# cslab-ntua/sparsex

Measured on AMD Instinct MI355X. Metric: SpMV GFLOP/s (2*nnz/t, alpha=0.5, x/y resident in HBM), higher is better.
Workload: dtype f64

## Files before the change

### include/sparsex_hip.h

```cpp
#ifndef SPARSEX_HIP_H
#define SPARSEX_HIP_H

#include <sparsex/sparsex.h>
#include <stdint.h>

#ifdef __cplusplus
extern "C" {
#endif

spx_error_t spx_hip_matvec_mult(spx_value_t alpha, const spx_matrix_t *A,
                                const spx_value_t *x_dev, spx_value_t *y_dev,
                                void *stream);
spx_error_t spx_hip_matvec_kernel(spx_value_t alpha, const spx_matrix_t *A,
                                  const spx_value_t *x_dev, spx_value_t beta,
                                  spx_value_t *y_dev, void *stream);

spx_error_t spx_hip_matvec_trans_mult(spx_value_t alpha, const spx_matrix_t *A,
                                      const spx_value_t *x_dev, spx_value_t *y_dev,
                                      void *stream);
spx_error_t spx_hip_matvec_trans_kernel(spx_value_t alpha, const spx_matrix_t *A,
                                        const spx_value_t *x_dev, spx_value_t beta,
                                        spx_value_t *y_dev, void *stream);
int spx_hip_matvec_trans_mode(const spx_matrix_t *A);

// ... 125 lines not shown
int spx_hip_mat_dist_parts(const spx_matrix_t *A);
spx_error_t spx_hip_mat_dist_round(const spx_matrix_t *A, int round, const size_t **send_off, const size_t **send_cnt,
                                   const size_t **recv_off, const size_t **recv_cnt);

typedef struct {
    int64_t nnz;
    int64_t nnz_stored;
    int64_t n_unit_elems;
    int64_t n_delta_elems;
    int64_t n_units;
    int64_t n_rowblocks;
    int64_t n_shared_rows;
    int64_t value_bytes;
    int64_t index_bytes;
    int32_t nr_partitions;
    int32_t first_partition, last_partition;
    int32_t row_lo, row_hi;
    int32_t symmetric;
    int32_t on_device;
    int32_t device;
    int32_t waves;
    int32_t sym_tiles;
    double  tune_seconds;
    double  emit_seconds;
    int32_t wave_tiles;
    int32_t sym_segments;
    int32_t quad;
    int32_t col_slices;
    int32_t unit_windows;
    int32_t unit_window_lds;
    int64_t unit_window_elems;
    int64_t unit_window_staged;
    int32_t sym_pipeline;
    int32_t reserved0;
    int64_t sym_pipeline_elems;
} spx_hip_info_t;

spx_error_t spx_hip_mat_info(const spx_matrix_t *A, spx_hip_info_t *info);

typedef struct {
    const uint32_t *tab;
    const uint32_t *xdescs;
    const void *passes;
    size_t n_rowblocks, n_descs, n_passes;
    size_t rowblocks_with_windows, rowblocks_with_units;
    uint64_t staged_doubles;
    uint64_t unit_elems, unit_elems_lds;
    uint32_t lds_doubles;
} spx_hip_xw_plan_t;
spx_error_t spx_hip_mat_unit_windows(spx_matrix_t *A, uint32_t budget, uint32_t gap, spx_hip_xw_plan_t *plan);

typedef struct {
    const void *passes;
    const uint32_t *n_sx;
    size_t n_rowblocks, n_passes;
    size_t rowblocks_with_sx;
    uint64_t sym_elems, sx_elems;
    uint64_t sym_passes, sx_passes;
} spx_hip_sx_plan_t;
spx_error_t spx_hip_mat_sym_pipeline(spx_matrix_t *A, spx_hip_sx_plan_t *plan);

spx_error_t spx_hip_mat_values_plan(spx_matrix_t *A, const spx_index_t *rowptr, const spx_index_t *colind, int indexing);
spx_error_t spx_hip_mat_values_plan_drop(spx_matrix_t *A);
spx_error_t spx_hip_mat_set_values(spx_matrix_t *A, const spx_value_t *values_dev, void *stream);
spx_error_t spx_hip_mat_set_values_host(spx_matrix_t *A, const spx_value_t *values);
typedef struct {
    const uint32_t *src_values;
// ... 65 lines not shown
```

### sparsex_amd/api.py

```python
import ctypes as C
import os

import numpy as np

SPX_SUCCESS = 0
SPX_FAILURE = -1
SPX_MAT_REORDER = 42
SPX_VEC_AS_IS = 43
SPX_VEC_TUNE = 44
SPX_INDEX_ZERO_BASED = 45
SPX_INDEX_ONE_BASED = 46

_HERE = os.path.dirname(os.path.abspath(__file__))


def lib_path():
    return os.environ.get("SPX_LIB_PATH") or os.path.join(_HERE, "lib", "libsparsex.so")


class SpxError(RuntimeError):
    pass


class VectorStruct(C.Structure):
    _fields_ = [("elements", C.POINTER(C.c_double)), ("size", C.c_size_t),
                ("alloc_type", C.c_int), ("vec_mode", C.c_int)]


class HipInfo(C.Structure):
    _fields_ = [("nnz", C.c_int64), ("nnz_stored", C.c_int64),
                ("n_unit_elems", C.c_int64), ("n_delta_elems", C.c_int64),
                ("n_units", C.c_int64), ("n_rowblocks", C.c_int64),
                ("n_shared_rows", C.c_int64), ("value_bytes", C.c_int64),
                ("index_bytes", C.c_int64), ("nr_partitions", C.c_int32),
                ("first_partition", C.c_int32), ("last_partition", C.c_int32),
                ("row_lo", C.c_int32), ("row_hi", C.c_int32),
                ("symmetric", C.c_int32), ("on_device", C.c_int32),
                ("device", C.c_int32), ("waves", C.c_int32), ("sym_tiles", C.c_int32),
                ("tune_seconds", C.c_double),
                ("emit_seconds", C.c_double), ("wave_tiles", C.c_int32), ("sym_segments", C.c_int32),
                ("quad", C.c_int32), ("col_slices", C.c_int32),
                ("unit_windows", C.c_int32), ("unit_window_lds", C.c_int32),
                ("unit_window_elems", C.c_int64), ("unit_window_staged", C.c_int64),
                ("sym_pipeline", C.c_int32), ("reserved0", C.c_int32), ("sym_pipeline_elems", C.c_int64)]


class SxPlan(C.Structure):
    _fields_ = [("passes", C.c_void_p), ("n_sx", C.POINTER(C.c_uint32)), ("n_rowblocks", C.c_size_t),
                ("n_passes", C.c_size_t), ("rowblocks_with_sx", C.c_size_t), ("sym_elems", C.c_uint64),
                ("sx_elems", C.c_uint64), ("sym_passes", C.c_uint64), ("sx_passes", C.c_uint64)]


class ValuesPlan(C.Structure):
    _fields_ = [("src_values", C.POINTER(C.c_uint32)), ("src_mirror", C.POINTER(C.c_uint32)),
                ("src_diag", C.POINTER(C.c_uint32)), ("n_values", C.c_size_t), ("n_mirror", C.c_size_t),
                ("n_diag", C.c_size_t), ("n_sources", C.c_uint64), ("n_dest", C.c_uint64),
                ("plan_bytes", C.c_uint64)]


class DiagPlan(C.Structure):
    _fields_ = [("pos", C.POINTER(C.c_uint32)), ("n_rows", C.c_size_t), ("row_lo", C.c_size_t),
                ("n_present", C.c_uint64), ("plan_bytes", C.c_uint64)]


class XwPlan(C.Structure):
    _fields_ = [("tab", C.POINTER(C.c_uint32)), ("xdescs", C.POINTER(C.c_uint32)), ("passes", C.c_void_p),
                ("n_rowblocks", C.c_size_t), ("n_descs", C.c_size_t), ("n_passes", C.c_size_t),
                ("rowblocks_with_windows", C.c_size_t), ("rowblocks_with_units", C.c_size_t),
                ("staged_doubles", C.c_uint64), ("unit_elems", C.c_uint64), ("unit_elems_lds", C.c_uint64),
                ("lds_doubles", C.c_uint32)]


class CsxExport(C.Structure):
    _fields_ = [("values", C.POINTER(C.c_double)), ("ctl", C.POINTER(C.c_uint8)),
                ("ctl_size", C.c_int64), ("nnz", C.c_int), ("ncols", C.c_int),
                ("nrows", C.c_int), ("row_start", C.c_int),
                ("row_jumps", C.c_int32), ("full_colind", C.c_int32),
# ... 999 lines not shown
```

### sparsex_amd/csrc/api.cpp

```cpp
#include <sparsex/sparsex.h>
#include <sparsex_hip.h>

#include "config.hpp"
#include "csx_emit.hpp"
#include "device.hpp"
#include "dist.hpp"
#include "encoder.hpp"
#include "gpu_emit.hpp"
#include "input.hpp"
#include "reorder.hpp"
#include "stream_index.hpp"
#include "threads.hpp"

#include <chrono>
#include <cmath>
#include <cstdarg>
#include <cstdint>
#include <cstring>
#include <functional>
#include <memory>
#include <mutex>
#include <atomic>
#include <sstream>
#include <thread>
// ... 333 lines not shown
{
    for (const SpxRowBlock &rb : s.rbs)
        for (uint32_t k = 0; k < rb.n_pass; ++k) {
            const uint8_t kind = s.passes[(size_t) rb.pass_off + k].kind;
            if (kind == SPX_PASS_SYMTILE || kind == SPX_PASS_SYMSEG) return true;
        }
    return false;
}

static void keep_index(spx_matrix_t *A, GpuStream &&gs)
{
    ValVec().swap(gs.values);
    std::vector<val_t>().swap(gs.dvalues);
    std::vector<val_t>().swap(gs.mirror_val);
    std::vector<uint32_t>().swap(gs.fix_idx);
    std::vector<uint32_t>().swap(gs.fix_ptr);
    std::vector<uint32_t>().swap(gs.spill_col);
    A->index.reset(new GpuStream(std::move(gs)));
}

constexpr size_t JOINED_ROWS = 1024, JOINED_ELEMS = 24576;
constexpr uint32_t JOINED_XW_BUDGET = 8192;

static size_t auto_target_elems(const spx_matrix_t *A, double scale)
{
    size_t local = 0;
    for (const Partition &p : A->parts) local += p.nnz * (A->symmetric ? 2 : 1);
    size_t t = std::min<size_t>(std::max<size_t>(local / 1280 + 1, 1024),
                                local > ((size_t) 64 << 20) ? SPX_MAX_RB_ELEMS : 4096);
    t = std::max<size_t>((size_t)(scale * (double) t), 512);
    return std::min<size_t>(t, SPX_MAX_RB_ELEMS);
}

static void emit_and_upload(spx_matrix_t *A)
{
    const size_t nown = A->parts.size();
    const size_t first = A->first_part;
    const bool sym = A->symmetric != 0;
    GpuEmitParams gp = A->emit_params;
    if (A->auto_rb) gp.target_elems = auto_target_elems(A, A->rb_scale);
    if (A->rb_joined) {
        gp.target_elems = JOINED_ELEMS;
        gp.max_rows = std::max<size_t>(gp.max_rows, JOINED_ROWS);
    }
    GpuStream gs;
    const unsigned hw = host_threads();
    struct Deferred {
        std::function<void()> f;
        ~Deferred() { if (f) f(); }
    } deferred;
    std::function<void()> &release_after_upload = deferred.f;
    const double t_emit0 = now_sec();
    auto emit_pieces = [&](std::vector<Partition> &pieces, const std::vector<std::vector<SymTile>> *tl,
                           const std::vector<SymSegVec> *sl = nullptr) {
        const size_t n = pieces.size();
        std::vector<GpuStream> locs(n);
        const unsigned inner = (unsigned) std::max<size_t>(1, hw / std::max<size_t>(1, std::min<size_t>(n, hw)));
        const double t_pieces = now_sec();
        parallel_for(n, hw, [&](size_t i) {
            GpuEmitParams g = gp;
            if (tl) g.tiles = &(*tl)[i];
            if (sl) g.symsegs = &(*sl)[i];
            emit_gpu(pieces[i], g, locs[i], inner);
        });
        const double t_room = now_sec();
        std::vector<uint64_t> v_at(n, UINT64_MAX);
        {
            size_t nv = gs.values.size(), nd = gs.descs.size(), np = gs.passes.size(), nc = gs.cidx.size(),
                   ns = gs.segrows.size(), nr = gs.rbs.size();
            for (size_t i = 0; i < n; ++i) {
                const GpuStream &l = locs[i];
                if (!(l.rbs.empty() && l.shared.empty())) {
                    nv += nv % 2;
                    v_at[i] = nv;
                    nv += l.values.size();
                }
// ... 138 lines not shown
                q.nr_rows = p.nr_rows; q.nr_cols = p.nr_cols; q.type = p.type; q.row_start = p.row_start;
                q.pool = p.pool;
                for (size_t e = 0; e < p.elems_size; ++e)
                    if (p.elems[e].col >= c_lo && p.elems[e].col < c_hi) {
                        q.elems.push_back(p.elems[e]);
                        q.nnz += p.elems[e].size;
                    }
                q.elems_size = q.elems.size();
            });
            gp.skip_empty = k > 0 || A->col_concurrent;
            const size_t rb0 = gs.rbs.size();
            emit_pieces(sub, nullptr);
            if (k > 0 && gs.rbs.size() > rb0) gs.rbs[rb0].flags |= SPX_RB_PHASE_START;
            if (A->col_concurrent && gs.rbs.size() == rb0) throw FatalError("column phases: an empty slice");
        }
        if (A->col_concurrent)
            for (SpxRowBlock &rb : gs.rbs) rb.flags |= SPX_RB_ACCUM;
        gp = keep;
        if (!gs.shared.empty()) throw FatalError("column phases: the matrix holds rows that are split over row-blocks");
    }
    const double t_emit1 = now_sec();
    A->conflict_rows.clear();
    if (sym && !gs.sym_fused) stream_touched_rows(gs, A->own_lo, A->conflict_rows);
    A->halo_cols.clear();
    if (A->own_lo > 0 || A->own_hi < A->nrows) stream_read_cols(gs, A->own_lo, A->own_hi, (size_t) A->ncols, A->halo_cols);
    A->first_block_row = A->own_lo;
    for (const SpxRowBlock &rb : gs.rbs) A->first_block_row = std::min<idx_t>(A->first_block_row, (idx_t) rb.row0);
    finalize_stream(gs, (size_t) A->nrows);
    if (sym) mark_private_rowblocks(gs, (size_t) A->nrows, A->own_lo, A->own_hi);
    std::vector<std::pair<uint32_t, uint32_t>>().swap(gs.direct_cols);
    gs.waves = (uint32_t) A->waves;
    gs.band_order = Config::instance().get_bool("spx.gpu.band_order");
    gs.arena = Config::instance().get_bool("spx.gpu.arena");
    gs.xw_budget = (A->unit_windows != 0 && !A->deterministic && !sym) ? (A->rb_joined ? std::max(A->xw_budget, JOINED_XW_BUDGET) : A->xw_budget) : 0u;
    gs.xw_gap = A->xw_gap;
    gs.xw_on = A->xw_on;
    gs.sx_plan = sym && A->sym_pipeline != 0 && !A->deterministic && A->wave_tiles != 1;
    gs.sx_on = A->sx_on;
    gs.sym_matmat = A->sym_matmat;
    gs.sym_atomic = A->sym_atomic && !A->deterministic;
    gs.deterministic = A->deterministic;
    gs.wave_tiles = A->deterministic || A->wave_tiles == 1;
    A->nnz_stored = gs.nnz_stored;
    A->n_unit_elems = gs.n_unit_elems;
    A->n_delta_elems = gs.n_delta_elems;
    A->n_units = gs.n_units;
    A->value_bytes = gs.values.size() * sizeof(val_t);
    A->index_bytes = gs.index_bytes();
    A->n_rowblocks = gs.rbs.size();
    A->n_shared = gs.shared.size();
    A->has_tiles = stream_has_tiles(gs);
    A->has_symtiles = stream_has_pass(gs, SPX_PASS_SYMTILE);
    if (A->dev) {
        device_free(A->dev);
        A->dev = nullptr;
    }
    const double t_emit2 = now_sec();
    if (!A->host_only) {
        A->dev = device_upload(gs, (size_t) A->nrows, (size_t) A->ncols, sym, A->own_lo, A->own_hi,
                               A->device_ordinal);
        device_set_trans_windows(A->dev, A->trans_windows);
        log_msg(LOG_INFO, "descriptor stream: emitted in %.2f s, finalized in %.2f s, uploaded in %.2f s (%zu row-blocks)\n",
                t_emit1 - t_emit0, t_emit2 - t_emit1, now_sec() - t_emit2, gs.rbs.size());
        if (A->dist && sym) {
            device_set_init_rows(A->dev, (size_t) dist_first_init_row(*A));
        }
        keep_index(A, std::move(gs));
// ... 17 lines not shown
    auto best_time = [&]() {
        A->release_wait();
        double best = device_time_spmv(A->dev, W, N);
        for (int rep = 0; rep < 3; ++rep) best = std::min(best, device_time_spmv(A->dev, 0, N));
        return best;
    };
    auto time_xw = [&](bool &xw) {
        if (!tune_xw || !device_has_xw(A->dev) || A->wave_tiles == 1) {
            xw = device_get_xw(A->dev);
            return best_time();
        }
        device_set_xw(A->dev, false);
        const double t0 = best_time();
        device_set_xw(A->dev, true);
        const double t1 = best_time();
        xw = t1 < 0.985 * t0;
        device_set_xw(A->dev, xw);
        return std::min(t0, xw ? t1 : t0);
    };
    if (!tune_waves) {
        if (tune_wave_tiles && !device_has_tiles(A->dev) && !(A->unit_windows == 1 && device_has_xw(A->dev))) {
            auto t_of = [&](bool on) {
                device_set_wave_tiles(A->dev, on);
                return best_time();
            };
            const double t0 = t_of(false), t1 = t_of(true);
            A->wave_tiles = t1 < 0.985 * t0 ? 1 : 0;
            device_set_wave_tiles(A->dev, A->wave_tiles == 1);
        }
        if (tune_xw && device_has_xw(A->dev) && A->wave_tiles != 1) {
            bool xw = false;
            (void) time_xw(xw);
            A->xw_on = xw;
        }
        if (!tune_spill || !device_has_spill(A->dev)) return;
        auto t_of = [&](bool atomic) {
            device_set_sym_atomic(A->dev, atomic);
            return best_time();
        };
        const double tl = t_of(false), ta = t_of(true);
        A->sym_atomic = ta < 0.985 * tl;
        device_set_sym_atomic(A->dev, A->sym_atomic);
        return;
    }
    auto time_with = [&](int waves, bool &xw) {
        device_set_waves(A->dev, waves);
        return time_xw(xw);
    };
    bool xw4 = false, xw8 = false;
    const double t4 = time_with(4, xw4), t8 = time_with(8, xw8);
    int best_waves = t8 < 0.985 * t4 ? 8 : 4;
    bool best_xw = best_waves == 8 ? xw8 : xw4;
    double best_t = std::min(t4, t8), best_scale = 1.0;
    device_set_xw(A->dev, best_xw);
    A->xw_on = best_xw;
    if (tune_wave_tiles && !device_has_tiles(A->dev) && !(A->unit_windows == 1 && device_has_xw(A->dev))) {
        device_set_wave_tiles(A->dev, true);
        device_set_waves(A->dev, best_waves);
        const double tw = best_time();
        if (tw < 0.985 * best_t) {
            best_t = tw;
            A->wave_tiles = 1;
            best_xw = false;
            A->xw_on = false;
        } else {
            device_set_wave_tiles(A->dev, false);
// ... 3 lines not shown
    }
    if (tune_spill && device_has_spill(A->dev)) {
        device_set_sym_atomic(A->dev, !A->sym_atomic);
        device_set_waves(A->dev, best_waves);
        const double ta = best_time();
        if (ta < 0.985 * best_t) {
            best_t = ta;
            A->sym_atomic = !A->sym_atomic;
        } else {
            device_set_sym_atomic(A->dev, A->sym_atomic);
        }
    }
    if (A->auto_rb && A->n_rowblocks <= 4096) {
        for (double scale : {0.7, 0.52}) {
            A->rb_scale = scale;
            A->waves = 2;
            emit_and_upload(A);
            bool xw2 = false;
            const double t2 = time_with(2, xw2);
            if (t2 < 0.985 * best_t) {
                best_t = t2;
                best_waves = 2;
                best_scale = scale;
                best_xw = xw2;
            }
        }
        A->xw_on = best_xw;
        if (A->rb_scale != best_scale) {
            A->rb_scale = best_scale;
            A->waves = best_waves;
            emit_and_upload(A);
        }
    }
    if (A->auto_rb && A->n_rowblocks > 4096 &&
        auto_target_elems(A, 2.0) != auto_target_elems(A, best_scale)) {
        A->rb_scale = 2.0;
        A->waves = best_waves;
        emit_and_upload(A);
        bool xwb = false;
        const double tb = time_with(best_waves, xwb);
        if (tb < 0.985 * best_t) {
            best_t = tb;
            best_scale = 2.0;
            best_xw = xwb;
            A->xw_on = best_xw;
        } else {
            A->rb_scale = best_scale;
            A->xw_on = best_xw;
            emit_and_upload(A);
        }
    }
    A->rb_scale = best_scale;
    A->waves = best_waves;
    A->xw_on = best_xw;
    if (A->auto_rb && best_xw && A->wave_tiles != 1 && A->emit_params.max_rows <= SPX_MAX_RB_ROWS &&
        A->value_bytes > ((size_t) 1 << 30)) {
        A->rb_joined = true;
        A->waves = 8;
        emit_and_upload(A);
        bool xwj = false;
        const double tj = time_with(8, xwj);
        if (xwj && tj < 0.995 * best_t) {
            best_t = tj;
            best_waves = 8;
            log_msg(LOG_INFO, "launch autotune: row-blocks joined side by side (%zu of them)\n", A->n_rowblocks);
        } else {
            A->rb_joined = false;
            A->waves = best_waves;
            A->xw_on = best_xw;
            emit_and_upload(A);
        }
    }
    A->waves = best_waves;
    A->xw_on = best_xw;
    device_set_waves(A->dev, best_waves);
    device_set_xw(A->dev, best_xw);
    log_msg(LOG_INFO, "launch autotune: %d wavefronts per workgroup, row-block scale %.2f%s, unit windows %s (%.2f us per SpMV)\n",
            best_waves, best_scale, A->rb_joined ? ", joined" : "", best_xw ? "on" : "off", 1e6 * best_t);
}

static int read_trans_windows()
{
    const std::string tw = Config::instance().get_str("spx.gpu.trans_windows");
    if (tw != "auto" && tw != "true" && tw != "false") {
        log_msg(LOG_ERR, "spx.gpu.trans_windows: true, false or auto\n");
        throw FatalError("bad spx.gpu.trans_windows");
    }
    return tw == "auto" ? -1 : (tw == "true" ? 1 : 0);
}

static int read_values_f32()
{
    const std::string v = Config::instance().get_str("spx.gpu.values_f32");
    if (v != "true" && v != "false" && v != "all") {
        log_msg(LOG_ERR, "spx.gpu.values_f32: false, true or all\n");
        throw FatalError("bad spx.gpu.values_f32");
    }
    return v == "all" ? 2 : (v == "true" ? 1 : 0);
}
static bool wants_values_f32(int mode, bool symmetric) { return mode == 2 || (mode == 1 && !symmetric); }

static spx_matrix_t *do_tune(spx_input_t *in)
{
    Config &cfg = Config::instance();
    const double t0 = now_sec();
    const size_t P = cfg.nr_partitions();
    long world = std::max<long>(1, cfg.get_long("spx.rt.gpu_world"));
    long rank = cfg.get_long("spx.rt.gpu_rank");
    if (rank < 0 || rank >= world || P % (size_t) world != 0) {
        log_msg(LOG_ERR, "spx.rt.gpu_rank/gpu_world (%ld/%ld) do not divide "
                "spx.rt.nr_threads=%zu partitions\n", rank, world, P);
// ... 183 lines not shown
        log_msg(LOG_ERR, "spx.gpu.unit_windows: true, false or auto\n");
        throw FatalError("bad spx.gpu.unit_windows");
    }
    {
        const long xb = cfg.get_long("spx.gpu.unit_window_doubles"), xg = cfg.get_long("spx.gpu.unit_window_gap");
        if (xb < 0 || xb > 16384 || xg < 0 || xg > 255) {
            log_msg(LOG_ERR, "spx.gpu.unit_window_doubles: 0 .. 16384, spx.gpu.unit_window_gap: 0 .. 255\n");
            throw FatalError("bad spx.gpu.unit_window_doubles / spx.gpu.unit_window_gap");
        }
        A->xw_budget = (uint32_t) xb;
        A->xw_gap = (uint32_t) xg;
    }
    A->unit_windows = xw_mode == "auto" ? -1 : (xw_mode == "true" ? 1 : 0);
    A->xw_on = xw_mode == "true";
    A->trans_windows = read_trans_windows();
    A->values_f32 = read_values_f32();
    const std::string sx_mode = cfg.get_str("spx.gpu.sym_pipeline");
    if (sx_mode != "auto" && sx_mode != "true" && sx_mode != "false") {
        log_msg(LOG_ERR, "spx.gpu.sym_pipeline: true, false or auto\n");
        throw FatalError("bad spx.gpu.sym_pipeline");
    }
    A->sym_pipeline = sx_mode == "auto" ? -1 : (sx_mode == "true" ? 1 : 0);
    A->sx_on = sx_mode == "true";
    const std::string ph_mode = cfg.get_str("spx.gpu.col_phases");
    const bool ph_conc = ph_mode.size() == 2 && ph_mode[0] == 'c';
    long ph_fixed = ph_mode == "auto" ? 0 : strtol(ph_mode.c_str() + (ph_conc ? 1 : 0), nullptr, 10);
    if (ph_mode != "auto" && (ph_fixed < 1 || ph_fixed > 8 || (ph_conc && ph_fixed != 2 && ph_fixed != 4 && ph_fixed != 8))) {
        log_msg(LOG_ERR, "spx.gpu.col_phases: 1 .. 8 (launched in turn), c2 | c4 | c8 (one launch, a group of XCDs each) or auto\n");
        throw FatalError("bad spx.gpu.col_phases");
    }
    A->col_phases = (!sym && ph_fixed > 1) ? (size_t) ph_fixed : 1;
    A->col_concurrent = A->col_phases > 1 && ph_conc && !A->deterministic;
    if (A->col_phases > 1 && ph_conc && !A->col_concurrent) A->col_phases = 1;
    try {
        emit_and_upload(A.get());
    } catch (const FatalError &) {
        if (A->col_phases <= 1) throw;
        A->col_phases = 1;
        emit_and_upload(A.get());
    }
    const bool tune_spill = spill_mode == "auto" && !A->deterministic && !A->has_symsegs && !A->sym_matmat;
    const bool tune_wt = wt_mode == "auto" && !A->deterministic && !A->has_symsegs;
    const bool tune_xw = xw_mode == "auto" && !A->deterministic && !sym;
    const double t_auto = now_sec();
    if (A->dev && A->nnz_stored >= 100000 && (autotune || tune_spill || tune_wt || tune_xw))
        autotune_launch(A.get(), autotune, tune_spill, tune_wt, tune_xw);
    if (A->dev && sym && A->sym_pipeline == -1 && device_has_sx(A->dev)) {
        A->release_wait();
        const double t_est = device_time_spmv(A->dev, 2, 3);
        const int N = (int) std::min(100.0, std::max(8.0, 0.02 / std::max(t_est, 1e-7)));
        auto best_of = [&](bool on) {
            device_set_sx(A->dev, on);
            double best = device_time_spmv(A->dev, std::max(2, N / 10), N);
            for (int rep = 0; rep < 3; ++rep) best = std::min(best, device_time_spmv(A->dev, 0, N));
            return best;
        };
        const double t0 = best_of(false), t1 = best_of(true);
        A->sx_on = t1 < 0.985 * t0;
        device_set_sx(A->dev, A->sx_on);
        log_msg(LOG_INFO, "read-once pipeline: %s (%.2f us per SpMV with, %.2f without)\n", A->sx_on ? "on" : "off", 1e6 * t1, 1e6 * t0);
    }
    const double t_auto_end = now_sec();
    if (A->dev && !sym && ph_mode == "auto" && A->n_shared == 0 && A->nnz_stored >= 100000 &&
        2 * A->n_delta_elems >= A->nnz_stored && (size_t) A->ncols * sizeof(val_t) >= ((size_t) 6 << 20)) {
        auto best_of = [&]() {
            double best = device_time_spmv(A->dev, 10, 100);
// ... 1420 lines not shown
} SPX_C_BOUNDARY(return SPX_FAILURE;)

spx_error_t spx_hip_mat_info(const spx_matrix_t *A, spx_hip_info_t *info)
try {
    if (!A || !info) { SETERROR_1(SPX_ERR_ARG_INVALID, "invalid argument"); return SPX_FAILURE; }
    memset(info, 0, sizeof(*info));
    info->nnz = A->nnz;
    info->nnz_stored = (int64_t) A->nnz_stored;
    info->n_unit_elems = (int64_t) A->n_unit_elems;
    info->n_delta_elems = (int64_t) A->n_delta_elems;
    info->n_units = (int64_t) A->n_units;
    info->n_rowblocks = (int64_t) A->n_rowblocks;
    info->n_shared_rows = (int64_t) A->n_shared;
    info->value_bytes = (int64_t) A->value_bytes;
    info->index_bytes = (int64_t) A->index_bytes;
    info->nr_partitions = (int32_t) A->nr_partitions;
    info->first_partition = (int32_t) A->first_part;
    info->last_partition = (int32_t) A->last_part;
    info->row_lo = A->own_lo;
    info->row_hi = A->own_hi;
    info->symmetric = A->symmetric;
    info->on_device = A->dev ? 1 : 0;
    if (A->dev) {
        DeviceMatrixInfo di;
        device_info(A->dev, di);
        info->device = di.device;
    }
    info->waves = A->dev ? device_get_waves(A->dev) : A->waves;
    info->sym_tiles = A->has_tiles ? ((A->dev ? device_get_sym_atomic(A->dev) : A->sym_atomic) ? 2 : 1) : 0;
    info->wave_tiles = A->dev ? (device_get_wave_tiles(A->dev) ? 1 : 0) : (A->wave_tiles == 1 || A->deterministic ? 1 : 0);
    info->sym_segments = A->has_symsegs ? (A->has_symtiles ? 1 : 2) : 0;
    info->col_slices = A->col_phases > 1 ? (A->col_concurrent ? (int32_t) A->col_phases : -(int32_t) A->col_phases) : 1;
    info->quad = 0;
    if (A->dev && device_has_xw(A->dev)) {
        uint64_t el = 0, ue = 0, st = 0;
        uint32_t lds = 0;
        device_xw_info(A->dev, el, ue, st, lds);
        info->unit_windows = device_get_xw(A->dev) ? 1 : 0;
        info->unit_window_lds = (int32_t) lds;
        info->unit_window_elems = (int64_t) el;
        info->unit_window_staged = (int64_t) st;
    }
    if (A->dev && device_has_sx(A->dev)) {
        uint64_t esx = 0, esym = 0;
        size_t nrb = 0;
        device_sx_info(A->dev, esx, esym, nrb);
        info->sym_pipeline = device_get_sx(A->dev) ? 1 : 0;
        info->sym_pipeline_elems = (int64_t) esx;
    }
    info->tune_seconds = A->tune_seconds;
    info->emit_seconds = A->emit_seconds;
    return SPX_SUCCESS;
} SPX_C_BOUNDARY(return SPX_FAILURE;)

static bool owned_part(const spx_matrix_t *A, int part)
{
    return part >= (int) A->first_part && part < (int) A->last_part &&
           (size_t)(part - (int) A->first_part) < A->parts.size();
}

spx_error_t spx_hip_mat_export_csx(const spx_matrix_t *A_, int part, spx_csx_export_t *out)
try {
    spx_matrix_t *A = const_cast<spx_matrix_t *>(A_);
    if (!A || !out) { SETERROR_1(SPX_ERR_ARG_INVALID, "invalid argument"); return SPX_FAILURE; }
    if (!owned_part(A, part)) {
        SETERROR_1(SPX_ERR_ARG_INVALID, "partition not held by this process "
// ... 323 lines not shown
```

### sparsex_amd/csrc/config.cpp

```cpp
#include "config.hpp"

#include <cstdlib>
#include <regex>
#include <sstream>

namespace spx {

Config &Config::instance()
{
    static Config c;
    return c;
}

Config::Config() { reset_defaults(); }

void Config::reset_defaults()
{
    props_.clear();
    props_["spx.rt.nr_threads"] = "1";
    props_["spx.rt.cpu_affinity"] = "0";
    props_["spx.preproc.heuristic"] = "ratio";
    props_["spx.preproc.xform"] = "all";
    props_["spx.preproc.sampling"] = "portion";
    props_["spx.preproc.sampling.nr_samples"] = "48";
    props_["spx.preproc.sampling.portion"] = "0.01";
    props_["spx.preproc.sampling.window_size"] = "0";
    props_["spx.matrix.symmetric"] = "false";
    props_["spx.matrix.split_blocks"] = "true";
    props_["spx.matrix.full_colind"] = "false";
    props_["spx.matrix.min_unit_size"] = "4";
    props_["spx.matrix.max_unit_size"] = "255";
    props_["spx.matrix.min_coverage"] = "0.1";
    props_["spx.matrix.onedim_blocks"] = "false";
    props_["spx.rt.host_only"] = "false";
    props_["spx.rt.gpu_rank"] = "0";
    props_["spx.rt.gpu_world"] = "1";
    props_["spx.rt.device"] = "-1";
    props_["spx.vec.register"] = "auto";
    props_["spx.vec.device"] = "false";
    props_["spx.rt.host_parts"] = "0";
    props_["spx.rt.dist_chunks"] = "4";
    props_["spx.rt.dist_reorder"] = "none";
    props_["spx.rt.row_offset"] = "0";
    props_["spx.rt.global_rows"] = "0";
    props_["spx.rt.keep_encoded"] = "true";
    props_["spx.gpu.rowblock_elems"] = "0";
    props_["spx.gpu.rowblock_rows"] = "512";
    props_["spx.gpu.stack_segments"] = "true";
    props_["spx.gpu.waves"] = "0";
    props_["spx.gpu.inline_desc"] = "true";
    props_["spx.gpu.arena"] = "false";
    props_["spx.gpu.band_order"] = "false";
    props_["spx.gpu.col_phases"] = "auto";
    props_["spx.gpu.keep_units"] = "true";
    props_["spx.gpu.recut_linear"] = "true";
    props_["spx.gpu.sym_once"] = "true";
    props_["spx.gpu.deterministic"] = "false";
    props_["spx.gpu.wave_tiles"] = "auto";
    props_["spx.gpu.x_window"] = "true";
    props_["spx.gpu.sym_segments"] = "auto";
    props_["spx.gpu.sym_segment_min"] = "2";
    props_["spx.gpu.sym_segment_max"] = "8";
    props_["spx.gpu.sym_wide_rows"] = "1024";
    props_["spx.gpu.sym_spill"] = "auto";
    props_["spx.gpu.sym_matmat"] = "false";
    props_["spx.gpu.sym_remine"] = "true";
    props_["spx.gpu.sym_pure_passes"] = "true";
    props_["spx.gpu.sym_pipeline"] = "auto";
    props_["spx.gpu.unit_windows"] = "auto";
    props_["spx.gpu.unit_window_doubles"] = "3072";
    props_["spx.gpu.unit_window_gap"] = "16";
    props_["spx.gpu.values_f32"] = "false";
    props_["spx.gpu.trans_windows"] = "auto";
}

bool Config::set(const std::string &key, const std::string &value)
{
    auto it = props_.find(key);
    if (it == props_.end()) {
        log_msg(LOG_WARN, "mnemonic \"%s\" not found\n", key.c_str());
// ... 138 lines not shown
```

### sparsex_amd/csrc/gpu_emit.cpp

```cpp
#include "gpu_emit.hpp"
#include "threads.hpp"

#include <algorithm>
#include <iterator>
#include <cassert>
#include <cstring>
#include <chrono>

namespace spx {

namespace {

struct Piece {
    uint32_t elem;
    uint16_t a, b;
};

struct Single { idx_t row, col; val_t val; };
typedef std::vector<Single, BigAlloc<Single>> SingleVec;
struct RowSeg { idx_t row, col; uint8_t width; val_t v[SPX_MAX_SEG_WIDTH]; };

template <class V, class KeyOf, class Within>
void sort_by_key_then(V &v, KeyOf key_of, Within within)
{
// ... 1237 lines not shown
    for (size_t i = 0; i < s.rbs.size(); ++i) {
        SpxRowBlock &rb = s.rbs[i];
        std::copy(s.passes.begin() + rb.pass_off, s.passes.begin() + rb.pass_off + rb.n_pass,
                  strided.begin() + i * (size_t) stride);
        rb.pass_off = (uint32_t)(i * (size_t) stride);
    }
    s.passes.swap(strided);
    s.pass_stride = stride;
}

void mark_private_rowblocks(GpuStream &s, size_t nrows, idx_t own_lo, idx_t own_hi)
{
    std::vector<char> touched(nrows + 8, 0);
    for (uint32_t g : s.slot_group_col)
        for (uint32_t c = g; c < g + 8; ++c) touched[c] = 1;
    for (const auto &d : s.direct_cols)
        for (uint32_t c = d.first; c < d.first + d.second && c < nrows; ++c) touched[c] = 1;
    for (uint32_t r : s.mirror_rows) touched[r] = 1;
    std::vector<uint32_t> upto(nrows + 1, 0);
    for (size_t r = 0; r < nrows; ++r) upto[r + 1] = upto[r] + (touched[r] ? 1u : 0u);
    for (SpxRowBlock &rb : s.rbs) {
        rb.flags &= (uint8_t) ~SPX_RB_PRIVATE;
        const size_t lo = rb.row0, hi = (size_t) rb.row0 + rb.n_rows;
        if ((rb.flags & SPX_RB_SHARED) || (idx_t) lo < own_lo || (idx_t) hi > own_hi || hi > nrows) continue;
        if (upto[hi] == upto[lo]) rb.flags |= SPX_RB_PRIVATE;
    }
}

void emit_gpu(const Partition &p, const GpuEmitParams &prm, GpuStream &out, unsigned nthreads)
{
    assert(p.type == ENC_H);
    const idx_t nrows = (idx_t) p.nr_rows;
    if (nrows == 0) return;
    const size_t max_rows = std::min<size_t>(prm.max_rows, SPX_MAX_RB_ROWS);
    const size_t target = std::min<size_t>(std::max<size_t>(prm.target_elems, 64),
                                           SPX_MAX_RB_ELEMS);

    std::vector<uint32_t> cnt((size_t) nrows, 0);
    for (size_t i = 0; i < p.elems_size; ++i) {
        const Elem &e = p.elems[i];
        if (!e.is_unit()) { ++cnt[(size_t) e.row - 1]; continue; }
        for (size_t k = 0; k < e.size; ++k) {
            idx_t r, c;
            unit_elem_coords(e, k, r, c);
            assert(r >= 1 && r <= nrows);
            ++cnt[(size_t) r - 1];
        }
    }
    static const std::vector<SymTile> no_tiles;
    const std::vector<SymTile> &tiles = prm.tiles ? *prm.tiles : no_tiles;
    for (const SymTile &t : tiles)
        for (idx_t r = 0; r < 8; ++r) cnt[(size_t)(t.row0 - p.row_start + r)] += 8;
    static const SymSegVec no_segs;
    const SymSegVec &symsegs = prm.symsegs ? *prm.symsegs : no_segs;
    for (const SymSeg &sg : symsegs) cnt[(size_t)(sg.row - p.row_start)] += sg.width;

    std::vector<char> tile_group((size_t) nrows / 8 + 2, 0);
    const idx_t g0 = p.row_start / 8;
    for (const SymTile &t : tiles) tile_group[(size_t)(t.row0 / 8 - g0)] = 1;
    auto in_group = [&](idx_t r) { return tile_group[(size_t)((p.row_start + r) / 8 - g0)] != 0; };
    std::vector<Plan> plans;
    {
        idx_t start = 0;
        size_t acc = 0;
        for (idx_t r = 0; r < nrows; ++r) {
            size_t c = cnt[(size_t) r];
            if (c > SPX_MAX_RB_ELEMS) {
                if (in_group(r)) throw FatalError("symmetric tile on an over-long row");
// ... 170 lines not shown
            }
            a = b;
        }
    };

    std::vector<std::vector<const SymTile *>> rb_tiles(plans.size());
    for (const SymTile &t : tiles) {
        const size_t r = (size_t)(t.row0 - p.row_start);
        const uint32_t pl = plan_of_row[r];
        if (plan_of_row[r + 7] != pl || plans[pl].split)
            throw FatalError("symmetric tile cut by a row-block border");
        rb_tiles[pl].push_back(&t);
    }

    std::vector<std::vector<const SymSeg *>> rb_segs(plans.size());
    for (const SymSeg &sg : symsegs) {
        const uint32_t pl = plan_of_row[(size_t)(sg.row - p.row_start)];
        if (plans[pl].split) throw FatalError("read-once segment on an over-long row");
        rb_segs[pl].push_back(&sg);
    }

    std::vector<std::pair<size_t, size_t>> jobs;
    {
        const size_t wide_seg = std::min<size_t>(prm.wide_rows, SPX_MAX_WIDE_ROWS);
        const size_t wide_any = std::min<size_t>(prm.max_rows, SPX_MAX_WIDE_ROWS);
        auto elems_of = [&](size_t i) {
            size_t e = 0;
            for (idx_t r = plans[i].row_lo; r < plans[i].row_hi; ++r) e += cnt[(size_t) r];
            return e;
        };
        auto joinable = [&](size_t i, bool seg) {
            if (plans[i].split || !rb_tiles[i].empty()) return false;
            return seg ? wide_seg > SPX_MAX_RB_ROWS && !rb_segs[i].empty()
                       : wide_any > SPX_MAX_RB_ROWS && rb_segs[i].empty();
        };
        for (size_t i = 0; i < plans.size();) {
            size_t j = i + 1;
            if (joinable(i, true)) {
                const idx_t row0g = p.row_start + plans[i].row_lo;
                auto seg_groups = [&](size_t q, std::vector<idx_t> &g) {
                    g.clear();
                    for (const SymSeg *sg : rb_segs[q])
                        for (idx_t c = sg->col & ~(idx_t) 7; c < sg->col + sg->width && c < row0g; c += 8) g.push_back(c);
                    std::sort(g.begin(), g.end());
                    g.erase(std::unique(g.begin(), g.end()), g.end());
                };
                std::vector<idx_t> uni, g, merged;
                seg_groups(i, uni);
                while (j < plans.size() && joinable(j, true) &&
                       (size_t)(plans[j].row_hi - plans[i].row_lo) <= wide_seg) {
                    seg_groups(j, g);
                    merged.clear();
                    std::set_union(uni.begin(), uni.end(), g.begin(), g.end(), std::back_inserter(merged));
                    if (merged.size() * 8 > SPX_MAX_WIDE_SLOTS) break;
                    uni.swap(merged);
                    ++j;
                }
            } else if (joinable(i, false)) {
                size_t e = elems_of(i);
                const size_t join_target = std::max<size_t>(target, std::min<size_t>(prm.target_elems, 4 * SPX_MAX_RB_ELEMS));
                while (j < plans.size() && joinable(j, false) &&
                       (size_t)(plans[j].row_hi - plans[i].row_lo) <= wide_any &&
                       e + elems_of(j) <= join_target + elems_of(j) / 2) {
                    e += elems_of(j);
                    ++j;
                }
            }
// ... 65 lines not shown
```

### sparsex_amd/csrc/gpu_emit.hpp

```cpp
#pragma once

#include "gpu_format.h"
#include "partition.hpp"

#include <utility>
#include <vector>

namespace spx {

struct SymTile {
    idx_t row0, col0;
    val_t v[64];
};

struct SymSeg {
    idx_t row, col;
    uint8_t width;
    val_t v[8];
};
typedef std::vector<SymSeg, BigAlloc<SymSeg>> SymSegVec;

struct GpuStream {
    ValVec values;
    std::vector<SpxUnitDesc> descs;
// ... 19 lines not shown
    uint32_t n_spill = 0;
    uint32_t lds_doubles = SPX_MAX_RB_ROWS;
    uint32_t pass_stride = 0;
    uint32_t waves = 4;
    bool band_order = false;
    bool arena = false;
    uint32_t xw_budget = 0, xw_gap = 16;
    bool xw_on = false;
    bool sx_plan = false, sx_on = false;
    bool sym_matmat = false;
    size_t nnz_stored = 0;
    size_t n_unit_elems = 0;
    size_t n_delta_elems = 0;
    size_t n_units = 0;

    size_t n_pass_used() const
    {
        size_t n = 0;
        for (const SpxRowBlock &rb : rbs) n += rb.n_pass;
        return n;
    }
    size_t index_bytes() const
    {
        return descs.size() * sizeof(SpxUnitDesc) + n_pass_used() * sizeof(SpxPass) + cidx.size() +
               (sym_atomic ? slot_group_col.size() : fix_ptr.size() + fix_idx.size()) * 4 +
               (mirror_rows.size() + mirror_ptr.size() + mirror_col.size()) * 4 +
               segrows.size() * 2 + rbs.size() * sizeof(SpxRowBlock);
    }
};

struct GpuEmitParams {
    size_t target_elems = 2048;
    size_t max_rows = SPX_MAX_RB_ROWS;
    size_t sym_min_run = 2;
    size_t sym_max_run = SPX_MAX_SEG_WIDTH;
    size_t wide_rows = SPX_MAX_RB_ROWS;
    bool skip_empty = false;
    bool stack_segments = true;
    bool recut_linear = true;
    bool inline_desc = true;
    bool keep_units = true;
    bool sym_remine = true;
    bool x_window = true;
    int sym_segments = -1;
    bool sym_pure_passes = true;
    bool sym_once = true;
    const std::vector<SymTile> *tiles = nullptr;
    const SymSegVec *symsegs = nullptr;
};

void emit_gpu(const Partition &p, const GpuEmitParams &prm, GpuStream &out, unsigned nthreads = 1);

void append_stream(GpuStream &dst, GpuStream &&src, uint64_t values_placed_at = UINT64_MAX);

void finalize_stream(GpuStream &s, size_t nrows);

void mark_private_rowblocks(GpuStream &s, size_t nrows, idx_t own_lo, idx_t own_hi);

void append_sym_expanded(const Partition &lower, Partition &out, bool remine_upper = true);

struct SymRange { idx_t lo, hi; };
struct MirrorPoint { idx_t row, col; val_t val; };
void build_sym_ranges(const std::vector<Partition> &lowers, const std::vector<SymRange> &ranges,
                      bool want_tiles, std::vector<Partition> &outs,
                      std::vector<std::vector<SymTile>> &tiles, unsigned nthreads,
                      std::vector<MirrorPoint> *sparse_mirror = nullptr,
// ... 24 lines not shown
```

### sparsex_amd/csrc/handles.hpp

```cpp
#pragma once

#include <sparsex/sparsex.h>
#include <sparsex_hip.h>

#include "csx_emit.hpp"
#include "device.hpp"
#include "gpu_emit.hpp"
#include "input.hpp"
#include "xwindows.hpp"
#include "sxplan.hpp"
#include "values_plan.hpp"
#include "diag_plan.hpp"

#include <algorithm>
#include <functional>
#include <memory>
#include <mutex>
#include <string>
#include <vector>
#include <thread>

namespace spx { struct DistPlan; }

using namespace spx;
// ... 39 lines not shown
    }
    ~matrix() { release_wait(); }
    std::vector<std::vector<val_t>> diag;
    std::vector<std::unique_ptr<CsxStream>> exported;
    std::vector<std::vector<spx_index_t>> exported_rows_info;
    bool full_colind = false;
    DeviceMatrix *dev = nullptr;
    std::unique_ptr<GpuStream> host_stream;
    std::unique_ptr<GpuStream> index;
    idx_t own_lo = 0, own_hi = 0;
    std::vector<idx_t> conflict_rows;
    std::vector<idx_t> halo_cols;
    idx_t first_block_row = 0;
    spx::DistPlan *dist = nullptr;
    GpuEmitParams emit_params;
    bool auto_rb = false;
    double rb_scale = 1.0;
    int waves = 4;
    size_t col_phases = 1;
    bool col_concurrent = false;
    bool host_only = false;
    bool has_tiles = false;
    bool sym_atomic = false;
    bool deterministic = false;
    bool has_symtiles = false;
    bool has_symsegs = false;
    int spill_mode = -1;
    bool sym_matmat = false;
    int wave_tiles = -1;
    int unit_windows = -1;
    bool xw_on = false;
    int values_f32 = 0;
    int trans_windows = -1;
    bool rb_joined = false;
    int sym_pipeline = -1;
    bool sx_on = false;
    uint32_t xw_budget = 3072, xw_gap = 16;
    std::unique_ptr<spx::XwPlan> xw_inspect;
    std::unique_ptr<spx::SxPlan> sx_inspect;
    std::unique_ptr<spx::ValuesPlan> values_plan;
    size_t values_plan_bytes = 0;
    bool values_refreshed = false;
    std::unique_ptr<spx::DiagPlan> diag_plan;
    size_t diag_plan_bytes = 0;
    spx::ValuesDigest pre_refresh_digest;
    bool has_pre_refresh_digest = false, edited_while_stale = false;
    int64_t input_row_base = -1;
    int device_ordinal = -1;
    std::vector<std::vector<idx_t>> spans;
    std::vector<idx_t> max_span;
    size_t nnz_stored = 0, n_unit_elems = 0, n_delta_elems = 0, n_units = 0;
    size_t value_bytes = 0, index_bytes = 0, n_rowblocks = 0, n_shared = 0;
    double tune_seconds = 0.0, emit_seconds = 0.0;
    std::string log;
    std::mutex mtx;
};

inline idx_t dist_first_init_row(const matrix &A)
{
    idx_t first = A.first_block_row;
    if (A.conflict_rows.empty()) return first;
    if (A.has_tiles) first = std::min(first, A.conflict_rows.front());
    return std::max(first, std::min(A.conflict_rows.front(), A.own_lo));
}
```

Baseline: 1170.

## Replace post-tune joined row-block trial with upfront sampled-unit-share row-block rule

Adds a row-block planning rule that runs before emission. For large general matrices, it samples rows to estimate the share of nonzeros stored in unit elements and chooses joined row-blocks when that share is high. It also adds a mode for explicit long row-blocks split into parts. This replaces the old approach of emitting and timing a joined layout after autotuning, with a fallback to planned row-blocks if unit windows lose. It avoids the extra emit and timing pass, but a threshold-based decision may pick the wrong layout for some matrices.

```diff
diff --git a/include/sparsex_hip.h b/include/sparsex_hip.h
--- a/include/sparsex_hip.h
+++ b/include/sparsex_hip.h
@@ -181,7 +181,7 @@
     int64_t unit_window_elems;
     int64_t unit_window_staged;
     int32_t sym_pipeline;
-    int32_t reserved0;
+    int32_t rowblock_plan;
     int64_t sym_pipeline_elems;
 } spx_hip_info_t;
 
diff --git a/sparsex_amd/api.py b/sparsex_amd/api.py
--- a/sparsex_amd/api.py
+++ b/sparsex_amd/api.py
@@ -42,7 +42,7 @@
                 ("quad", C.c_int32), ("col_slices", C.c_int32),
                 ("unit_windows", C.c_int32), ("unit_window_lds", C.c_int32),
                 ("unit_window_elems", C.c_int64), ("unit_window_staged", C.c_int64),
-                ("sym_pipeline", C.c_int32), ("reserved0", C.c_int32), ("sym_pipeline_elems", C.c_int64)]
+                ("sym_pipeline", C.c_int32), ("rowblock_plan", C.c_int32), ("sym_pipeline_elems", C.c_int64)]
 
 
 class SxPlan(C.Structure):
diff --git a/sparsex_amd/csrc/api.cpp b/sparsex_amd/csrc/api.cpp
--- a/sparsex_amd/csrc/api.cpp
+++ b/sparsex_amd/csrc/api.cpp
@@ -389,6 +389,96 @@
     return std::min<size_t>(t, SPX_MAX_RB_ELEMS);
 }
 
+struct RowblockRuleInput {
+    size_t value_bytes = 0;
+    size_t min_bytes = 0;
+    double unit_share = 0.0;
+};
+
+constexpr double LONG_RB_UNIT_SHARE = 0.9;
+
+static spx_matrix_t::RowblockPlan long_rowblocks(uint32_t rows, double nnz_per_row, uint32_t budget)
+{
+    spx_matrix_t::RowblockPlan pl;
+    const double want = std::max(64.0, nnz_per_row * (double) rows);
+    const uint32_t n_parts = (uint32_t) std::max(2.0, std::ceil(want / (double) SPX_MAX_RB_ELEMS));
+    pl.rows = rows;
+    pl.part_rows = std::max<uint32_t>(rows / n_parts, 8);
+    pl.part_elems = (uint32_t) std::min<double>(SPX_MAX_RB_ELEMS, std::ceil(want / n_parts));
+    pl.elems = pl.part_elems * n_parts;
+    pl.xw_budget = budget;
+    return pl;
+}
+
+static spx_matrix_t::RowblockPlan joined_rowblocks()
+{
+    spx_matrix_t::RowblockPlan pl;
+    pl.rows = (uint32_t) JOINED_ROWS;
+    pl.elems = (uint32_t) JOINED_ELEMS;
+    pl.xw_budget = JOINED_XW_BUDGET;
+    return pl;
+}
+
+static bool rowblock_rule_decide(const RowblockRuleInput &in)
+{
+    return in.value_bytes > in.min_bytes && in.unit_share >= LONG_RB_UNIT_SHARE;
+}
+
+static void rowblock_rule(spx_matrix_t *A, const std::string &mode, size_t min_bytes)
+{
+    A->rb_plan = spx_matrix_t::RowblockPlan();
+    const bool general_xw = !A->symmetric && A->unit_windows != 0 && !A->deterministic && A->wave_tiles != 1 &&
+                            A->col_phases <= 1;
+    if (mode == "plain" || !general_xw || !A->auto_rb || A->emit_params.max_rows != SPX_MAX_RB_ROWS) return;
+    size_t nnz = 0, rows = 0;
+    for (const Partition &p : A->parts) {
+        nnz += p.nnz;
+        rows += p.nr_rows;
+    }
+    if (nnz == 0 || rows == 0) return;
+    if (mode == "joined") {
+        A->rb_plan = joined_rowblocks();
+    } else if (mode != "auto") {
+        A->rb_plan = long_rowblocks((uint32_t) strtol(mode.c_str(), nullptr, 10), (double) nnz / (double) rows, A->xw_budget);
+    } else {
+        RowblockRuleInput in;
+        in.value_bytes = nnz * sizeof(val_t);
+        in.min_bytes = min_bytes;
+        if (in.value_bytes <= in.min_bytes) return;
+        const size_t n_samples = std::min<size_t>(A->parts.size(), 8);
+        std::vector<uint64_t> in_units(n_samples, 0), in_all(n_samples, 0);
+        parallel_for(n_samples, host_threads(), [&](size_t s) {
+            const Partition &p = A->parts[s * A->parts.size() / n_samples];
+            const idx_t last = (idx_t) p.rowptr.size() - 1;
+            for (idx_t q = 1; q < 8; q += 2) {
+                const idx_t lo = std::max<idx_t>(0, (idx_t) ((int64_t) last * q / 8) - 128), hi = std::min<idx_t>(last, lo + 256);
+                for (idx_t r = lo; r < hi; ++r)
+                    for (idx_t j = p.rowptr[(size_t) r]; j < p.rowptr[(size_t) r + 1]; ++j) {
+                        const Elem &e = p.elems[(size_t) j];
+                        in_all[s] += e.size;
+                        if (e.is_unit()) in_units[s] += e.size;
+                    }
+            }
+        });
+        uint64_t ue = 0, all = 0;
+        for (size_t s = 0; s < n_samples; ++s) {
+            ue += in_units[s];
+            all += in_all[s];
+        }
+        in.unit_share = all ? (double) ue / (double) all : 0.0;
+        if (rowblock_rule_decide(in)) {
+            A->rb_plan = joined_rowblocks();
+            A->rb_plan.by_rule = true;
+        }
+        log_msg(LOG_INFO, "row-block size rule: %.2f GB of values, %.0f %% of the sampled nonzeros in units -> %s row-blocks\n",
+                in.value_bytes / 1e9, 100.0 * in.unit_share, A->rb_plan.rows ? "joined" : "planned");
+    }
+    if (A->rb_plan.rows)
+        log_msg(LOG_INFO, "row-blocks of up to %u rows and %u nonzeros (parts of %u nonzeros, window budget %u doubles)\n",
+                A->rb_plan.rows, A->rb_plan.elems, A->rb_plan.part_elems ? A->rb_plan.part_elems : (uint32_t) SPX_MAX_RB_ELEMS,
+                std::max(A->xw_budget, A->rb_plan.xw_budget));
+}
+
 static void emit_and_upload(spx_matrix_t *A)
 {
     const size_t nown = A->parts.size();
@@ -396,9 +486,11 @@
     const bool sym = A->symmetric != 0;
     GpuEmitParams gp = A->emit_params;
     if (A->auto_rb) gp.target_elems = auto_target_elems(A, A->rb_scale);
-    if (A->rb_joined) {
-        gp.target_elems = JOINED_ELEMS;
-        gp.max_rows = std::max<size_t>(gp.max_rows, JOINED_ROWS);
+    if (A->rb_plan.rows) {
+        gp.target_elems = A->rb_plan.elems;
+        gp.max_rows = A->rb_plan.rows;
+        gp.part_elems = A->rb_plan.part_elems;
+        gp.part_rows = A->rb_plan.part_rows;
     }
     GpuStream gs;
     const unsigned hw = host_threads();
@@ -603,7 +695,7 @@
     gs.waves = (uint32_t) A->waves;
     gs.band_order = Config::instance().get_bool("spx.gpu.band_order");
     gs.arena = Config::instance().get_bool("spx.gpu.arena");
-    gs.xw_budget = (A->unit_windows != 0 && !A->deterministic && !sym) ? (A->rb_joined ? std::max(A->xw_budget, JOINED_XW_BUDGET) : A->xw_budget) : 0u;
+    gs.xw_budget = (A->unit_windows != 0 && !A->deterministic && !sym) ? std::max(A->xw_budget, A->rb_plan.xw_budget) : 0u;
     gs.xw_gap = A->xw_gap;
     gs.xw_on = A->xw_on;
     gs.sx_plan = sym && A->sym_pipeline != 0 && !A->deterministic && A->wave_tiles != 1;
@@ -687,6 +779,12 @@
             bool xw = false;
             (void) time_xw(xw);
             A->xw_on = xw;
+        }
+        if (A->rb_plan.by_rule && !A->xw_on) {
+            A->rb_plan = spx_matrix_t::RowblockPlan();
+            emit_and_upload(A);
+            autotune_launch(A, tune_waves, tune_spill, tune_wave_tiles, tune_xw);
+            return;
         }
         if (!tune_spill || !device_has_spill(A->dev)) return;
         auto t_of = [&](bool atomic) {
@@ -756,7 +854,7 @@
             emit_and_upload(A);
         }
     }
-    if (A->auto_rb && A->n_rowblocks > 4096 &&
+    if (A->auto_rb && A->n_rowblocks > 4096 && A->rb_plan.rows == 0 &&
         auto_target_elems(A, 2.0) != auto_target_elems(A, best_scale)) {
         A->rb_scale = 2.0;
         A->waves = best_waves;
@@ -777,30 +875,21 @@
     A->rb_scale = best_scale;
     A->waves = best_waves;
     A->xw_on = best_xw;
-    if (A->auto_rb && best_xw && A->wave_tiles != 1 && A->emit_params.max_rows <= SPX_MAX_RB_ROWS &&
-        A->value_bytes > ((size_t) 1 << 30)) {
-        A->rb_joined = true;
-        A->waves = 8;
+    if (A->rb_plan.by_rule && !best_xw) {
+        log_msg(LOG_INFO, "launch autotune: unit windows lose on the joined row-blocks (%.2f us per SpMV): planned row-blocks\n", 1e6 * best_t);
+        A->rb_plan = spx_matrix_t::RowblockPlan();
+        A->rb_scale = 1.0;
+        A->waves = 4;
         emit_and_upload(A);
-        bool xwj = false;
-        const double tj = time_with(8, xwj);
-        if (xwj && tj < 0.995 * best_t) {
-            best_t = tj;
-            best_waves = 8;
-            log_msg(LOG_INFO, "launch autotune: row-blocks joined side by side (%zu of them)\n", A->n_rowblocks);
-        } else {
-            A->rb_joined = false;
-            A->waves = best_waves;
-            A->xw_on = best_xw;
-            emit_and_upload(A);
-        }
+        autotune_launch(A, tune_waves, tune_spill, tune_wave_tiles, tune_xw);
+        return;
     }
     A->waves = best_waves;
     A->xw_on = best_xw;
     device_set_waves(A->dev, best_waves);
     device_set_xw(A->dev, best_xw);
     log_msg(LOG_INFO, "launch autotune: %d wavefronts per workgroup, row-block scale %.2f%s, unit windows %s (%.2f us per SpMV)\n",
-            best_waves, best_scale, A->rb_joined ? ", joined" : "", best_xw ? "on" : "off", 1e6 * best_t);
+            best_waves, best_scale, A->rb_plan.rows ? ", long row-blocks" : "", best_xw ? "on" : "off", 1e6 * best_t);
 }
 
 static int read_trans_windows()
@@ -1050,6 +1139,22 @@
     A->col_phases = (!sym && ph_fixed > 1) ? (size_t) ph_fixed : 1;
     A->col_concurrent = A->col_phases > 1 && ph_conc && !A->deterministic;
     if (A->col_phases > 1 && ph_conc && !A->col_concurrent) A->col_phases = 1;
+    {
+        const std::string rp_mode = cfg.get_str("spx.gpu.rowblock_plan");
+        char *end = nullptr;
+        const long rp_rows = strtol(rp_mode.c_str(), &end, 10);
+        const bool number = end != rp_mode.c_str() && *end == '\0';
+        if (number ? (rp_rows < 64 || rp_rows > SPX_MAX_WIDE_ROWS) : (rp_mode != "auto" && rp_mode != "plain" && rp_mode != "joined")) {
+            log_msg(LOG_ERR, "spx.gpu.rowblock_plan: auto, plain, joined or 64 .. %d rows\n", SPX_MAX_WIDE_ROWS);
+            throw FatalError("bad spx.gpu.rowblock_plan");
+        }
+        const long rp_min = cfg.get_long("spx.gpu.rowblock_plan_min_bytes");
+        if (rp_min < 0) {
+            log_msg(LOG_ERR, "spx.gpu.rowblock_plan_min_bytes: 0 or more\n");
+            throw FatalError("bad spx.gpu.rowblock_plan_min_bytes");
+        }
+        rowblock_rule(A.get(), rp_mode, (size_t) rp_min);
+    }
     try {
         emit_and_upload(A.get());
     } catch (const FatalError &) {
@@ -2536,6 +2641,7 @@
     info->sym_segments = A->has_symsegs ? (A->has_symtiles ? 1 : 2) : 0;
     info->col_slices = A->col_phases > 1 ? (A->col_concurrent ? (int32_t) A->col_phases : -(int32_t) A->col_phases) : 1;
     info->quad = 0;
+    info->rowblock_plan = (int32_t) A->rb_plan.rows;
     if (A->dev && device_has_xw(A->dev)) {
         uint64_t el = 0, ue = 0, st = 0;
         uint32_t lds = 0;
diff --git a/sparsex_amd/csrc/config.cpp b/sparsex_amd/csrc/config.cpp
--- a/sparsex_amd/csrc/config.cpp
+++ b/sparsex_amd/csrc/config.cpp
@@ -46,6 +46,8 @@
     props_["spx.rt.keep_encoded"] = "true";
     props_["spx.gpu.rowblock_elems"] = "0";
     props_["spx.gpu.rowblock_rows"] = "512";
+    props_["spx.gpu.rowblock_plan"] = "auto";
+    props_["spx.gpu.rowblock_plan_min_bytes"] = "1073741824";
     props_["spx.gpu.stack_segments"] = "true";
     props_["spx.gpu.waves"] = "0";
     props_["spx.gpu.inline_desc"] = "true";
diff --git a/sparsex_amd/csrc/gpu_emit.cpp b/sparsex_amd/csrc/gpu_emit.cpp
--- a/sparsex_amd/csrc/gpu_emit.cpp
+++ b/sparsex_amd/csrc/gpu_emit.cpp
@@ -1293,8 +1293,8 @@
     assert(p.type == ENC_H);
     const idx_t nrows = (idx_t) p.nr_rows;
     if (nrows == 0) return;
-    const size_t max_rows = std::min<size_t>(prm.max_rows, SPX_MAX_RB_ROWS);
-    const size_t target = std::min<size_t>(std::max<size_t>(prm.target_elems, 64),
+    const size_t max_rows = std::min<size_t>(prm.part_elems && prm.part_rows ? prm.part_rows : prm.max_rows, SPX_MAX_RB_ROWS);
+    const size_t target = std::min<size_t>(std::max<size_t>(prm.part_elems ? prm.part_elems : prm.target_elems, 64),
                                            SPX_MAX_RB_ELEMS);
 
     std::vector<uint32_t> cnt((size_t) nrows, 0);
@@ -1531,7 +1531,7 @@
         auto joinable = [&](size_t i, bool seg) {
             if (plans[i].split || !rb_tiles[i].empty()) return false;
             return seg ? wide_seg > SPX_MAX_RB_ROWS && !rb_segs[i].empty()
-                       : wide_any > SPX_MAX_RB_ROWS && rb_segs[i].empty();
+                       : (wide_any > SPX_MAX_RB_ROWS || prm.part_elems != 0) && rb_segs[i].empty();
         };
         for (size_t i = 0; i < plans.size();) {
             size_t j = i + 1;
diff --git a/sparsex_amd/csrc/gpu_emit.hpp b/sparsex_amd/csrc/gpu_emit.hpp
--- a/sparsex_amd/csrc/gpu_emit.hpp
+++ b/sparsex_amd/csrc/gpu_emit.hpp
@@ -75,6 +75,8 @@
 struct GpuEmitParams {
     size_t target_elems = 2048;
     size_t max_rows = SPX_MAX_RB_ROWS;
+    size_t part_elems = 0;
+    size_t part_rows = 0;
     size_t sym_min_run = 2;
     size_t sym_max_run = SPX_MAX_SEG_WIDTH;
     size_t wide_rows = SPX_MAX_RB_ROWS;
diff --git a/sparsex_amd/csrc/handles.hpp b/sparsex_amd/csrc/handles.hpp
--- a/sparsex_amd/csrc/handles.hpp
+++ b/sparsex_amd/csrc/handles.hpp
@@ -95,7 +95,10 @@
     bool xw_on = false;
     int values_f32 = 0;
     int trans_windows = -1;
-    bool rb_joined = false;
+    struct RowblockPlan {
+        uint32_t rows = 0, elems = 0, part_elems = 0, part_rows = 0, xw_budget = 0;
+        bool by_rule = false;
+    } rb_plan;
     int sym_pipeline = -1;
     bool sx_on = false;
     uint32_t xw_budget = 3072, xw_gap = 16;
```

New measurement: 1178, median of 5. Within noise of the previous version (+0.7%).
